# underactuated/HSLabs

Measured on AMD Instinct MI355X. Metric: batched control-loop steps/sec (hexapod.xml, 18-DoF) at 1/2/4/8 MI355X, higher is better.
Workload: dtype f64

## Files before the change

hslabs_amd/api.py:

```python
from __future__ import annotations

import ctypes
from dataclasses import dataclass, field

import numpy as np

from . import capi

GAIT_DTYPE = np.dtype([
    ("torso_pos", "<f8", (3,)), ("torso_angles", "<f8", (3,)), ("step_duration", "<f8"),
    ("period", "<f8"), ("step_length", "<f8"), ("step_height", "<f8"), ("curvature", "<f8"),
    ("foot_shift", "<f8"), ("foot_shift_type", "<i4"), ("rec_transform_flag", "<i4"),
    ("rec_transl", "<f8", (3,)), ("rec_eas", "<f8", (3,)), ("reserved", "<f8", (5,)),
])
assert GAIT_DTYPE.itemsize == 192


def _require(ok: bool, msg: str) -> None:
    if not ok:
        raise ValueError(msg)

SWEEP_NAMES = ("step_duration", "period", "step_length", "step_height")


# ... 141 lines not shown
    def __del__(self):
        try:
            if self.handle:
                capi.load().hs_model_free(self.handle)
                self.handle = None
        except Exception:
            pass


def limb_tile_launches() -> int:
    return int(capi.load().hs_limb_tile_launches())


def limb_tile_plan_launches() -> int:
    return int(capi.load().hs_limb_tile_plan_launches())


def limb_launches() -> int:
    return int(capi.load().hs_limb_launches())


def limb_deferred() -> int:
    d = ctypes.c_int64()
    capi.check(capi.load().hs_limb_stats(None, ctypes.byref(d)), "hs_limb_stats")
    return int(d.value)


def params_array(params) -> np.ndarray:
    if isinstance(params, np.ndarray) and params.dtype == GAIT_DTYPE:
        return np.ascontiguousarray(params)
# ... 724 lines not shown
```

hslabs_amd/capi.py:

```python
from __future__ import annotations

import ctypes
import hashlib
import os

from . import build as _build

ABI_VERSION = 16

HS_OK = 0
HS_FLAG_RANK_RETRY = 1
HS_FLAG_FULL_RANK = 2
HS_FLAG_LOOP_EXHAUST = 4
HS_FLAG_NAN = 8
HS_FLAG_UNREACH = 16
HS_FLAG_NO_CONTACT = 32
HS_FLAG_GENERAL = 64
HS_FLAG_NEAR_RANK = 256
HS_FLAG_DEPENDENT = 512
HS_PREC_F64 = 0
HS_PREC_F32 = 1
HS_SOLVE_AUTO = 0
HS_SOLVE_REFERENCE = 1
KEY_MIN_STEP_LENGTH = 1e-3
# ... 1 lines not shown

EXPORTS = [
    "hs_model_load", "hs_model_load_ex", "hs_model_free", "hs_model_get_dims", "hs_pgs_config_read",
    "hs_run", "hs_run_steps", "hs_run_calls", "hs_run_pd", "hs_run_forces", "hs_run_forces_calls", "hs_mixed_create", "hs_mixed_free",
    "hs_mixed_get_dims", "hs_complete_traj", "hs_traj_save", "hs_run_forces_host",
    "hs_run_mixed", "hs_run_mixed_steps", "hs_run_mixed_calls", "hs_run_host", "hs_best_key_cot", "hs_best_key_encode",
    "hs_best_key_decode", "hs_last_error", "hs_abi_version",
    "hs_sim_default_params", "hs_sim_reset", "hs_sim_step", "hs_sim_create", "hs_sim_advance", "hs_sim_get_state",
    "hs_sim_free", "hs_sim_trial", "hs_sim_trial_summary", "hs_sim_set_trial", "hs_sim_get_trial_state",
    "hs_sim_config", "hs_sim_track_push", "hs_sim_probe", "hs_sim_estimate_workspace",
    "hs_batch_create", "hs_batch_set_params", "hs_batch_run", "hs_batch_run_device", "hs_select_best",
    "hs_batch_best_key_device", "hs_batch_free", "hs_comm_unique_id", "hs_comm_init", "hs_comm_free", "hs_comm_size",
    "hs_comm_reduce_best", "hs_select_best_comm", "hs_pergen_rec", "hs_pergen_rec_host", "hs_model_lik",
    "hs_model_lik_host", "hs_model_fk", "hs_model_fk_host", "hs_model_get_node", "hs_model_set_torso_penalty",
    "hs_model_get_torso_penalty", "hs_model_limb_lane", "hs_limb_launches", "hs_limb_tile_launches", "hs_limb_stats",
    "hs_limb_tile_plan_launches",
]
EXPORTS_B = ["hs_sim_regress_B", "hs_sim_estimate_B"]
HS_FLAG_LIK_FAILED = 128
SIM_BODY_STRIDE = 13
HS_TRIAL_RUNNING = -1
HS_TRIAL_SURVIVED = -2


class GaitParamsC(ctypes.Structure):

    _fields_ = [
        ("torso_pos", ctypes.c_double * 3),
        ("torso_angles", ctypes.c_double * 3),
        ("step_duration", ctypes.c_double),
        ("period", ctypes.c_double),
# ... 208 lines not shown
    L.hs_pergen_rec_host.argtypes = [vp, ctypes.POINTER(GaitParamsC), ctypes.c_int32, dp, ctypes.c_int32, dp]
    L.hs_model_lik.argtypes = [vp, ctypes.c_int32, vp, ctypes.c_int32, vp, vp, vp]
    L.hs_model_lik_host.argtypes = [vp, ctypes.c_int32, dp, ctypes.c_int32, dp, u32p]
    L.hs_model_fk.argtypes = [vp, ctypes.c_int32, vp, ctypes.c_int32, vp, vp, vp]
    L.hs_model_fk_host.argtypes = [vp, ctypes.c_int32, dp, ctypes.c_int32, dp, dp]
    L.hs_model_get_node.argtypes = [vp, ctypes.c_int32, ctypes.POINTER(NodeInfoC)]
    L.hs_last_error.argtypes = []
    L.hs_last_error.restype = ctypes.c_char_p
    L.hs_model_limb_lane.argtypes = [vp, ctypes.POINTER(ctypes.c_int32)]
    L.hs_limb_launches.argtypes = []
    L.hs_limb_launches.restype = ctypes.c_int64
    L.hs_limb_tile_launches.argtypes = []
    L.hs_limb_tile_launches.restype = ctypes.c_int64
    L.hs_limb_tile_plan_launches.argtypes = []
    L.hs_limb_tile_plan_launches.restype = ctypes.c_int64
    L.hs_limb_stats.argtypes = [ctypes.POINTER(ctypes.c_int64), ctypes.POINTER(ctypes.c_int64)]
    L.hs_abi_version.argtypes = []
    L.hs_abi_version.restype = ctypes.c_int
    if L.hs_abi_version() != ABI_VERSION:
        raise HSError("libhslabs ABI version mismatch")
    _lib = L
    return L


def check(rc: int, what: str = "") -> None:
    if rc != HS_OK:
        msg = load().hs_last_error().decode(errors="replace")
        raise HSError(f"{what}: {msg} (rc={rc})")
```

hslabs_amd/csrc/hs_capi.cpp:

```cpp
#include <hip/hip_runtime.h>

#include <algorithm>
#include <atomic>
#include <cmath>
#include <cstdio>
#include <cstdlib>
#include <cstring>
#include <fstream>
#include <mutex>
#include <string>
#include <vector>

#include "hs_internal.h"

namespace {

thread_local std::string g_err;

int fail(int code, const std::string& msg) {
  g_err = msg;
  return code;
}

}
// ... 252 lines not shown
    if (e != hipSuccess) return hip_fail(e, "hipEventRecord");
  }
  if (key_reduce) {
    hs_run_args r = c;
    r.best_key = a.best_key;
    r.accumulate = 1;
    const int le = k.launch_fused_reduce(r, cx.total_mass, cx.rollout_mass, nullptr, 0);
    if (le != 0) return hip_fail((hipError_t)le, "kernel launch (best key)");
  }
  return HS_OK;
}

std::atomic<int64_t> g_limb_launches{0};
std::atomic<int64_t> g_limb_tile_launches{0};
std::atomic<int64_t> g_limb_tile_plan_launches{0};
#define HS_ONLINE_MAX_H 64

bool env_switch(const char* name, bool on_by_default) {
  const char* e = getenv(name);
  if (!e) return on_by_default;
  return on_by_default ? e[0] != '0' : e[0] == '1';
}

enum class step_route {
  ROLLOUT,
  ONLINE_DEFER,
  LIMB_ONLINE,
  FUSED,
  LIMB_FUSED,
};
// ... 19 lines not shown
#endif
bool limb_tile(step_route rt, const hs_run_args& a, int32_t n) {
  if (rt != step_route::LIMB_FUSED || !env_switch("HS_LIMB_TILE", true)) return false;
  if (const char* e = getenv("HS_LIMB_TILE_MIN")) {
    char* end = nullptr;
    const long min_n = strtol(e, &end, 10);
    if (end != e && *end == '\0' && min_n >= 1) return n >= min_n;
  }
  const int32_t idle = HS_TILE_SLOTS * limb_tile_count(n) - n;
  return a.precision != HS_PREC_F32 && n >= HS_LIMB_TILE_MIN_STEPS && 32 * idle <= n;
}
int32_t limb_tile_plan_mode() {
  if (!env_switch("HS_LIMB_TILE_PLAN", true)) return 0;
  const char* e = getenv("HS_LIMB_TILE_PLAN");
  return e && e[0] == '2' ? 2 : 1;
}

#ifndef HS_FUSED_WAVES
#define HS_FUSED_WAVES 524288
#endif
#ifndef HS_FUSED_MAX_STEPS
#define HS_FUSED_MAX_STEPS 256
#endif
#ifndef HS_FUSED_RESERVE_STEPS
#define HS_FUSED_RESERVE_STEPS 1024
#endif
int32_t fused_chunk(const hs::launch_map& mp) {
  return std::max(1, std::min(HS_FUSED_MAX_STEPS, HS_FUSED_WAVES / std::max(1, mp.n_waves)));
}

// ... 48 lines not shown
  int le = launch_setup(cx, c, mp);
  mp.red_total_mass = cx.total_mass;
  mp.red_rollout_mass = cx.rollout_mass;
  mp.red_key_steps = r.key_steps;
  hipStream_t st = (hipStream_t)a.stream;
  for (int32_t i = 0; le == 0 && i < n_chunks; i++) {
    const int64_t s0 = online ? 0 : (int64_t)i * CHUNK;
    const bool last = i + 1 == n_chunks;
    if (online) c.k0 = (int32_t)(((int64_t)a.k0 + (int64_t)i * a.horizon) % a.n_t);
    mp.fused_s0 = (int32_t)s0;
    mp.fused_n = (int32_t)std::min<int64_t>(CHUNK, S - s0);
    mp.fix_mode = hs::FIX_DEFER;
    mp.fix_count = fix_counts + i;
    mp.fix_reduce = 0;
    mp.limb_tile = limb_tile(rt, a, mp.fused_n);
    hipError_t e = kernel_events ? hipEventRecord((hipEvent_t)kernel_events[2 * i], st) : hipSuccess;
    if (e != hipSuccess) return hip_fail(e, "hipEventRecord");
    int32_t planned = 0;
    le = limb ? k.launch_limb(cx.d_topo, c, cx.ws, mp, limb_tile_plan_mode(), &planned)
              : k.launch_fused(cx.d_topo, c, cx.ws, mp);
    g_limb_launches += limb;
    g_limb_tile_launches += mp.limb_tile;
    g_limb_tile_plan_launches += planned;
    if (le != 0) break;
    mp.fix_mode = hs::FIX_SOLVE;
    mp.fix_reduce = a.work_cot && a.solve_mode == HS_SOLVE_AUTO && (online || last);
    mp.fix_barrier = barrier_ok ? fix_counts + n_chunks + i : nullptr;
    mp.red_n_steps = (int32_t)S;
    mp.red_best_key = last ? r.best_key : nullptr;
    le = k.launch_fused(cx.d_topo, c, cx.ws, mp);
    if (le == 0 && kernel_events) e = hipEventRecord((hipEvent_t)kernel_events[2 * i + 1], st);
    if (e != hipSuccess) return hip_fail(e, "hipEventRecord");
  }
  if (le == 0 && !mp.fix_reduce) le = k.launch_fused_reduce(r, cx.total_mass, cx.rollout_mass, work, (int32_t)S);
  if (le != 0) return hip_fail((hipError_t)le, "kernel launch");
  return HS_OK;
}

// ... 16 lines not shown
}

extern "C" {

int hs_abi_version(void) { return HSLABS_ABI_VERSION; }

int hs_model_limb_lane(hs_model_t m, int32_t* ok) {
  if (!m || !ok) return fail(HS_E_ARG, "null argument");
  *ok = m->host.limb_lane_ok;
  return HS_OK;
}

int64_t hs_limb_launches(void) { return g_limb_launches.load(); }
int64_t hs_limb_tile_launches(void) { return g_limb_tile_launches.load(); }
int64_t hs_limb_tile_plan_launches(void) { return g_limb_tile_plan_launches.load(); }

int hs_limb_stats(int64_t* launches, int64_t* deferred) {
  if (launches) *launches = g_limb_launches.load();
  if (deferred) {
    unsigned long long n[2] = {0, 0};
    hipError_t e = (hipError_t)hs::kernels_f64.limb_deferred(&n[0]);
    if (e == hipSuccess) e = (hipError_t)hs::kernels_f32.limb_deferred(&n[1]);
    if (e != hipSuccess) return hip_fail(e, "hs_limb_stats");
    *deferred = (int64_t)(n[0] + n[1]);
  }
  return HS_OK;
}

const char* hs_last_error(void) { return g_err.c_str(); }

// ... 186 lines not shown
          (hipError_t)cx.pools->fused_fix.get(a->stream, (fix_bytes(n_chunks, CHUNK, mp) + gwb - 1) / gwb, &fix);
      if (e != hipSuccess) return hip_fail(e, "hipMalloc(forces fixup items)");
    }
    fix_counts = (int32_t*)fix;
    fix_carve(fix, n_chunks, mp);
    mp.prep_unit = 8;
  }
  int le = launch_setup(cx, c, mp);
  for (int64_t s0 = 0, ci = 0; le == 0 && s0 < S; s0 += CHUNK, ci++) {
    mp.fused_s0 = (int32_t)s0;
    mp.fused_n = (int32_t)std::min<int64_t>(CHUNK, S - s0);
    if (limb) {
      mp.fix_count = fix_counts + ci;
      mp.fix_mode = hs::FIX_DEFER;
      mp.limb_tile = limb_tile(step_route::LIMB_FUSED, *a, mp.fused_n);
      int32_t planned = 0;
      le = k.launch_limb(cx.d_topo, c, cx.ws, mp, limb_tile_plan_mode(), &planned);
      g_limb_launches++;
      g_limb_tile_launches += mp.limb_tile;
      g_limb_tile_plan_launches += planned;
      if (le != 0) break;
      mp.fix_mode = hs::FIX_SOLVE;
      mp.fix_reduce = 0;
      le = k.launch_fused(cx.d_topo, c, cx.ws, mp);
      mp.fix_mode = hs::FIX_NONE;
    } else {
      le = k.launch_fused(cx.d_topo, c, cx.ws, mp);
    }
  }
  if (le != 0) return hip_fail((hipError_t)le, "kernel launch");
// ... 1241 lines not shown
```

hslabs_amd/csrc/hs_internal.h:

```cpp
#pragma once
#include <cstddef>
#include <mutex>
#include <string>
#include <vector>

#include "../../include/hslabs.h"
#include "hs_simtopo.h"
#include "hs_limb_tile.h"
#include "hs_topo.h"

struct hs_sim_probe_kargs {
  hs_sim_args sim;
  int32_t m, pad;
  const double* tau0;
  const double* dtau;
  double* config_out;
  double* tau_out;
  double* body_out;
  uint32_t* seed_out;
};

namespace hs {

int set_error(int code, const std::string& msg);
// ... 25 lines not shown
  int32_t setup_only;
  int32_t fix_mode;
  int32_t* fix_count;
  int32_t* fix_items;
  int32_t fix_n_counts;
  int32_t fix_reduce, red_key_steps, red_n_steps;
  int32_t* fix_barrier;
  double red_total_mass;
  const double* red_rollout_mass;
  uint64_t* red_best_key;
  int32_t ktab_n, ktab_lo, ktab_nl, ttab_n;
  int32_t prep_unit;
  const int32_t *limb_model, *limb_rollouts, *limb_slots;
  int32_t limb_waves;
  int32_t limb_tile;
};

size_t solve_workspace_bytes();
void ktab_range(int32_t k0, int32_t n_t, int32_t horizon, int64_t n_calls, int32_t* lo, int32_t* n_table,
                int32_t* n_ttab);
launch_map single_model_map(const hs_topo& t, int32_t n_rollouts);

struct kernels {
  size_t (*general_workspace_bytes)();
  int (*launch_rollouts)(const hs_topo* d_topo, const hs_run_args& a, void* workspace, const launch_map& mp);
  int (*launch_fused)(const hs_topo* d_topo, const hs_run_args& a, void* workspace, const launch_map& mp);
  int (*launch_limb)(const hs_topo* d_topo, const hs_run_args& a, void* workspace, const launch_map& mp,
                     int32_t tile_plan, int32_t* tile_planned);
  int (*launch_fused_reduce)(const hs_run_args& a, double total_mass, const double* rollout_mass,
                             const void* work_steps, int32_t n_steps);
// ... 67 lines not shown
```

hslabs_amd/csrc/hs_kernels.hip:

```cpp
#include <hip/hip_runtime.h>

#include <cfloat>
#include <cstdint>
#include <type_traits>

#ifndef HS_REAL_IS_FLOAT
#define HS_REAL_IS_FLOAT 0
#endif
#include "hs_internal.h"
#include "hs_math.h"

namespace {

using namespace hsd;

#ifndef HS_CURVED_LDS
#define HS_CURVED_LDS HS_REAL_IS_FLOAT
#endif
#ifndef HS_PRELOAD
#define HS_PRELOAD (!HS_REAL_IS_FLOAT)
#endif
#ifndef HS_KTE_PRELOAD
#define HS_KTE_PRELOAD (!HS_REAL_IS_FLOAT)
#endif
// ... 172 lines not shown
template <class T>
__device__ inline bool near_thr(T v, T t, T band) { return v >= t / band && v <= t * band; }

__device__ inline real* outp(double* p) { return reinterpret_cast<real*>(p); }
__device__ inline const real* inp(const double* p) { return reinterpret_cast<const real*>(p); }

template <class G>
__device__ inline void gsync() {
  if constexpr (G::SHARED) wave_sync();
  else __syncthreads();
}

#ifdef HS_STAMPS
__device__ unsigned long long g_stamps[4096][32];
__device__ unsigned int g_stamp_base;
#define STAMP(slot)                                                                                    \
  do {                                                                                                 \
    const unsigned r_ = blockIdx.x - g_stamp_base;                                                     \
    if (threadIdx.x == 0 && r_ < 4096u) g_stamps[r_][slot] = __builtin_amdgcn_s_memtime();             \
  } while (0)
#define RSTAMP(slot)                                                                                   \
  do {                                                                                                 \
    const unsigned r_ = blockIdx.x - g_stamp_base;                                                     \
    if (threadIdx.x == 0 && r_ < 4096u) g_stamps[r_][slot] = __builtin_amdgcn_s_memrealtime();         \
  } while (0)
#else
#define STAMP(slot) do {} while (0)
#define RSTAMP(slot) do {} while (0)
#endif

#ifdef HS_DBG
__device__ double g_dbg[1 << 22];
__device__ inline int* dbg_rows() {
  __shared__ int r[8];
// ... 2861 lines not shown
extern "C" int hs_debug_read_dbg(double* out, int n) {
  if (n > (1 << 22)) n = 1 << 22;
  return (int)hipMemcpyFromSymbol(out, HIP_SYMBOL(g_dbg), sizeof(double) * n, 0, hipMemcpyDeviceToHost);
}
#endif

#if defined(HS_STAMPS) && !HS_REAL_IS_FLOAT
extern "C" int hs_debug_read_stamps(unsigned long long* out, int n_rows) {
  if (n_rows > 4096) n_rows = 4096;
  return (int)hipMemcpyFromSymbol(out, HIP_SYMBOL(g_stamps), sizeof(unsigned long long) * 32 * n_rows, 0,
                                  hipMemcpyDeviceToHost);
}
extern "C" int hs_debug_set_stamp_base(unsigned int base) {
  return (int)hipMemcpyToSymbol(HIP_SYMBOL(g_stamp_base), &base, sizeof(base), 0, hipMemcpyHostToDevice);
}
extern "C" int hs_debug_clear_stamps() {
  static unsigned long long zero[4096][32];
  return (int)hipMemcpyToSymbol(HIP_SYMBOL(g_stamps), zero, sizeof(zero), 0, hipMemcpyHostToDevice);
}
#endif

namespace hs {

static size_t general_workspace_bytes() { return sizeof(RolloutWS); }

static int limb_deferred(unsigned long long* out) {
  return (int)hipMemcpyFromSymbol(out, HIP_SYMBOL(g_limb_deferred), sizeof(unsigned long long), 0,
                                  hipMemcpyDeviceToHost);
}

// ... 82 lines not shown
  if (mp.max_parts <= 18) launch_nm<18>(d_topo, a, ws, m, st);
  else if (mp.max_parts <= 22) launch_nm<22>(d_topo, a, ws, m, st);
  else launch_nm<HS_NMAX>(d_topo, a, ws, m, st);
  return (int)hipGetLastError();
}

static int launch_limb(const hs_topo* d_topo, const hs_run_args& a, void* workspace, const launch_map& mp,
                       int32_t tile_plan, int32_t* tile_planned) {
  if (tile_planned) *tile_planned = 0;
  if (a.n_rollouts <= 0 || mp.fused_n <= 0) return 0;
  hipStream_t st = (hipStream_t)a.stream;
  RolloutWS* ws = (RolloutWS*)workspace;
  launch_map m = mp;
  m.fused_w = mp.limb_rollouts ? mp.limb_waves : (a.n_rollouts + LGR - 1) / LGR;
  const int vsteps = mp.limb_tile ? HS_TILE_SLOTS * limb_tile_count(mp.fused_n) : mp.fused_n;
  const dim3 grid((unsigned)((int64_t)m.fused_w * vsteps));
  const int nm = mp.max_parts <= 18 ? 18 : (mp.max_parts <= 22 ? 22 : HS_NMAX);
  limb_tile_plan_arg plan = {};
  if (mp.limb_tile && tile_plan && mp.fused_n <= HS_TILE_PLAN_STEPS && mp.fused_h >= 1 && a.n_t >= 1 && a.k0 >= 0 &&
      mp.fused_s0 >= 0) {
    const limb_tile_launch L = {mp.fused_n, mp.fused_s0, mp.fused_h, a.k0, a.n_t, mp.ktab_nl > 0 ? mp.ktab_nl : HS_LMAX};
    bool planned = true;
    if (tile_plan == 2) {
      int row[HS_TILE_PLAN_STEPS];
      limb_tile_rows(L, row);
      limb_tile_chain_fill(row, L.n, plan.step);
    } else {
      planned = limb_tile_plan(L, plan.step);
    }
    if (planned) plan.n_slots = vsteps;
    if (tile_planned) *tile_planned = planned;
// ... 47 lines not shown
```

hslabs_amd/csrc/hs_limb.h:

```cpp

#ifndef HS_LIMB_GROUP
#define HS_LIMB_GROUP HS_FUSED_GROUP
#endif
#ifndef HS_LIMB_WAVES
#define HS_LIMB_WAVES 2
#endif
#ifndef HS_LIMB_WAVES_F32
#define HS_LIMB_WAVES_F32 HS_LIMB_WAVES
#endif

constexpr int LG = 8;
constexpr int LGR = WAVE / LG;

__device__ unsigned long long g_limb_deferred;

template <int NM, bool FORCES = false>
struct LimbLds {
  real g[NM][6];
  real a[6];
  real wd[HS_NMAX];
  real p[FORCES ? NM : 1][3];
};

__device__ inline real grp_get(real v, int src) { return __shfl(v, src); }
// ... 169 lines not shown
      }
    }
    for (int e = 0; e < 6; e++) tD[m][e] = Dp[e];
    for (int i = 0; i < 3; i++) tg[m][i] = g[i];
  }
#pragma unroll
  for (int e = 0; e < 6; e++) Dp6[e] = (tD[0][e] + tD[1][e]) + (tD[2][e] + real(0));
#pragma unroll
  for (int i = 0; i < 3; i++) gc[i] = (tg[0][i] + tg[1][i]) + (tg[2][i] + real(0));
}

template <int NM>
__device__ __attribute__((always_inline)) inline void limb_forces(const hs_topo* T, const hs_run_args& a,
                                                                  const hs::launch_map& mp, LimbLds<NM, true>& S, bool limb,
                                                                  int l, int L, int gbase, int nl, bool live, int b,
                                                                  int fstep, int s_glob, const real* o,
                                                                  const real (&Jp)[3][3], const real (&Jz)[3][3],
                                                                  const real (&Pc)[3][3], const real* fp,
                                                                  const real (&xt)[3][3], bool bad, bool big) {
  const int n = T->n;
#ifdef HS_DBG
  const int dbg_r = live ? b * a.horizon + s_glob : -1;
#define FDBG(slot, val, n_)                                                                                      \
  do {                                                                                                           \
    if (HS_DBG == (n_) && dbg_r >= 0 && (size_t)dbg_r * 32 + (slot) < (1u << 22)) g_dbg[(size_t)dbg_r * 32 + (slot)] = (double)(val); \
  } while (0)
#else
#define FDBG(slot, val, n_) do {} while (0)
#endif
  real ts[9];
#pragma unroll
// ... 31 lines not shown
      for (int e = 0; e < 27; e++) {
        const TriWalk<> t(e < 21 ? e : 0);
        real pa = e < 21 ? F.prod(t.r, t.c) : F.prod(e - 21, 9);
        real pb = e < 21 ? G.vprod(t.r, t.c) : G.vprod(e - 21, 6);
        opaque_vals<1>(&pa);
        opaque_vals<1>(&pb);
        vl[e] = (e < 21) ? pb - pa : pb + pa;
      }
    }
  }
  const bool fast = !grp_any(limb && !okB, gbase);
  if (!fast || grp_any(big, gbase)) {
    if (l == 0 && live) {
      atomicAdd(&g_limb_deferred, 1ull);
      const int it = atomicAdd(mp.fix_count, 1);
      mp.fix_items[2 * it] = fstep;
      mp.fix_items[2 * it + 1] = b;
    }
    return;
  }
  real kv[27];
#pragma unroll
  for (int e = 0; e < 27; e++) {
    const real v = limb ? vl[e] : real(0);
    real s = real(0) + v;
    for (int k = 1; k < nl; k++) {
      const real prev = dpp_r<0x111>(s);
      if (l >= 1) s = prev + v;
    }
    const real tot = grp_get(s, gbase + nl - 1);
    const real dtv = (e < 21) ? real(0) : (e < 24 ? S.a[e - 21] : S.a[e - 21]);
// ... 53 lines not shown
    return (real)__hiloint2double(hi, lo);
  } else {
    return (real)__int_as_float(__builtin_amdgcn_ds_permute(dst << 2, __float_as_int((float)v)));
  }
}

#ifdef HS_DBG
#define TDBG(slot, val, n)                                                                                       \
  do {                                                                                                           \
    if (HS_DBG == (n) && dbg_r >= 0 && (size_t)dbg_r * 32 + (slot) < (1u << 22)) g_dbg[(size_t)dbg_r * 32 + (slot)] = (double)(val); \
  } while (0)
#else
#define TDBG(slot, val, n) do {} while (0)
#endif

template <bool FORCES>
__device__ __attribute__((always_inline)) inline void limb_tile_kd(
    const hs_topo* T_, real (&outer)[36][LGR * HS_LMAX], hs_link (&links)[HS_LMAX][3], const RolloutWS& W, bool straight,
    const real* u, real v, int lane, int nl, bool limb, int L, bool live, int row0, const real* tv, const real* o,
    real inv, real dt, real (&g3)[3][6], real (&Jp)[3][3], real (&Jz)[3][3], real* fp, bool& contact, bool& own,
    real* gown, real* jvel, real (&Pc)[3][3], real* Pown, bool& bad, bool& big, int dbg_r) {
  (void)dbg_r;
  const int grp = lane >> 3, l = lane & 7;
  const int rprev = __shfl(row0, (lane + WAVE - LG) & (WAVE - 1)), rnext = __shfl(row0, (lane + LG) & (WAVE - 1));
  const uint64_t lv = __ballot(live);
  const bool lprev = grp > 0 && ((lv >> ((lane - LG) & (WAVE - 1))) & 1);
  const bool lnext = grp < LGR - 1 && ((lv >> ((lane + LG) & (WAVE - 1))) & 1);
  const bool shm = live && lprev && rprev + 2 == row0;
  const bool shp = live && lnext && rnext == row0 + 2;
  uint32_t M = 0;
  {
    const uint64_t bm = __ballot(live && !shm), bp = __ballot(live && !shp);
#pragma unroll
    for (int g = 0; g < LGR; g++)
      M |= (uint32_t)((bm >> (LG * g)) & 1) << (2 * g) | (uint32_t)((bp >> (LG * g)) & 1) << (2 * g + 1);
  }
  const int nreq = __popc(M);
// ... 160 lines not shown
    for (int r = 0; r < 5; r += 2)
#pragma unroll
      for (int kk = 0; kk < 3; kk++) big |= sincos_big(W.ktab[row0 + r][L][kk]);
#pragma unroll
    for (int kk = 0; kk < 3; kk++) {
      if constexpr (FORCES) break;
      real dd = W.ktab[row0 + 3][L][kk] - W.ktab[row0 + 1][L][kk];
      if (dd > kPi) dd -= 2 * kPi;
      else if (dd < -kPi) dd += 2 * kPi;
      jvel[kk] = dd / (2 * dt);
    }
  }
}
#undef TDBG

template <int NM, bool FORCES, bool TILE = false, class... PLAN>
__global__ __launch_bounds__(WAVE, HS_REAL_IS_FLOAT ? HS_LIMB_WAVES_F32 : HS_LIMB_WAVES) void hs_limb_kernel(const hs_topo* __restrict__ T0, hs_run_args a,
                                                                      RolloutWS* __restrict__ rws, hs::launch_map mp, PLAN... plan) {
  static_assert(sizeof...(PLAN) == (TILE ? 1 : 0), "the tile mapping takes the launch's plan, the packed mapping nothing");
  __shared__ union {
    struct {
      real outer[36][LGR * HS_LMAX];
      hs_link links[HS_LMAX][3];
    } k;
    LimbLds<NM, FORCES> g[LGR];
  } sh;
  LimbLds<NM, FORCES>* lds = sh.g;
  int fstep = 0, q = (int)blockIdx.x;
  fused_coords<HS_LIMB_GROUP>((int)blockIdx.x, mp.fused_w, TILE ? HS_TILE_SLOTS * limb_tile_count(mp.fused_n) : mp.fused_n,
                              fstep, q);
  const hs_topo* __restrict__ T = mp.limb_model ? T0 + mp.limb_model[q] : T0;
  {
    const uint64_t* src = reinterpret_cast<const uint64_t*>(&T->link[0][0]);
    uint64_t* dst = reinterpret_cast<uint64_t*>(&sh.k.links[0][0]);
    constexpr int NW = sizeof(sh.k.links) / sizeof(uint64_t);
    for (int e = (int)threadIdx.x; e < NW; e += WAVE) dst[e] = src[e];
    wave_sync();
  }
  RSTAMP(16);
  STAMP(15);
  const int lane = (int)threadIdx.x, grp = lane >> 3, l = lane & 7, gbase = lane & ~7;
  const int rslot = q * LGR + (TILE ? fstep % LGR : grp);
  const int b = mp.limb_rollouts ? mp.limb_rollouts[rslot] : rslot;
  bool live = b >= 0 && b < a.n_rollouts;
  if constexpr (TILE) {
    if (!live) return;
    const int slot0 = HS_TILE_SLOTS * (fstep / LGR), ls = limb_tile_plan_step(plan..., slot0 + grp, mp.fused_n);
    live = ls >= 0;
    fstep = live ? ls : limb_tile_plan_step(plan..., slot0, mp.fused_n);
  }
  const int bb = live || TILE ? b : (mp.limb_rollouts ? mp.limb_rollouts[q * LGR] : a.n_rollouts - 1);
  LimbLds<NM, FORCES>& S = lds[grp];
  const int ol = grp * HS_LMAX + (l < HS_LMAX ? l : 0);
  const int s_glob = mp.fused_s0 + fstep, call = s_glob / mp.fused_h;
  const int k0 = (int)(((int64_t)a.k0 + (int64_t)call * mp.fused_h) % a.n_t) + s_glob % mp.fused_h;
  const int row0 = k0 - mp.ktab_lo;
  const int nl = T->n_limbs, nmj = T->nmj;
  const bool limb = l < nl, tlane = l == LG - 1;
  const int L = limb ? l : 0;
  const RolloutWS& W = rws[bb];
  const hs_gait_params& gp = a.params[bb];
  const bool straight = (real)gp.curvature == 0 && !gp.rec_transform_flag;
  const real dt = W.st.dt;
  const real v = W.st.v;
  const NodeK n0 = load_nodek(T, 0);
  const real u[3] = {n0.Jp(0, 0), n0.Jp(1, 0), n0.Jp(2, 0)};
  real tv[5];
#pragma unroll
  for (int k = 0; k < 5; k += 2) tv[k] = W.t_tab[row0 + k] * v;
  real o[3];
  if (straight) {
    for (int i = 0; i < 3; i++) o[i] = fma(tv[2], u[i], W.kf.torso[i]);
  } else {
    mulp(load34r(W.ktor[row0 + 2] + 6), n0.com, o);
  }
  const real inv = real(1) / (2 * dt);
#ifdef HS_DBG
  const int dbg_r = live ? b * a.horizon + s_glob : -1;
#define LDBG(slot, val, n)                                                                                       \
  do {                                                                                                           \
    if (HS_DBG == (n) && dbg_r >= 0 && (size_t)dbg_r * 32 + (slot) < (1u << 22)) g_dbg[(size_t)dbg_r * 32 + (slot)] = (double)(val); \
  } while (0)
#else
#define LDBG(slot, val, n) do {} while (0)
#endif

  real g0[6];
  {
    BodyS tb[3];
#pragma unroll
    for (int k = 0; k < 3; k++) {
      if (straight) tb[k] = body_straight(W.kf.torso, u, tv[2 * k]);
      else tb[k] = body_frame(load34r(W.ktor[row0 + 2 * k] + 6), n0.com);
    }
    part_dyn((real)T->mass[0], inv, tb[0].P, tb[1].P, tb[2].P, tb[0].U, tb[1].U, tb[2].U, g0);
    part_g(tb[1].P, o, g0);
  }
  STAMP(0);
  real g3[3][6];
  real Jp[3][3], Jz[3][3], fp[3];
  bool contact = false;
  bool own = false;
  real gown[6];
  real jvel[3];
  real Pc[3][3], Pown[3];
  bool bad = false, big = false;
  const hs_topo* const T_ = T;
  if constexpr (TILE) {
    limb_tile_kd<FORCES>(T_, sh.k.outer, sh.k.links, W, straight, u, v, lane, nl, limb, L, live, row0, tv, o, inv, dt, g3,
                         Jp, Jz, fp, contact, own, gown, jvel, Pc, Pown, bad, big, live ? b * a.horizon + s_glob : -1);
  } else if (limb) {
    const int row = row0;
    own = T->limb_own_n[L] > 0;
    BodyS om, op, oc;
    {
      real P[3][3], U[3][3];
      const hs_topo* Ts = opaque_s(T);
      limb_outer(Ts, sh.k.links[L], limb_frame(Ts, L, straight, own, W, row, u, tv[0], om), W.ktab[row][L], P, U, big);
#pragma unroll
      for (int kk = 0; kk < 3; kk++)
#pragma unroll
        for (int j = 0; j < 3; j++) {
          sh.k.outer[3 * kk + j][ol] = P[kk][j];
          sh.k.outer[9 + 3 * kk + j][ol] = U[kk][j];
        }
// ... 143 lines not shown
    const int nk = T->node[0].nkids;
    for (int kk = 0; kk < HS_CMAX; kk++) {
      if (kk >= nk) break;
      const int c = T->node[0].kids[kk];
      for (int j = 0; j < 3; j++) { F[j] += S.g[c][j]; V[j] += S.g[c][3 + j]; }
    }
    const real d[3] = {0, 0, 0};
    V[0] -= d[1] * F[2] - d[2] * F[1];
    V[1] -= d[2] * F[0] - d[0] * F[2];
    V[2] -= d[0] * F[1] - d[1] * F[0];
    for (int j = 0; j < 3; j++) { S.a[j] = F[j]; S.a[3 + j] = V[j]; }
  }
  wave_sync();

  STAMP(5);
  if constexpr (FORCES) {
    limb_forces<NM>(T, a, mp, S, limb, l, L, gbase, nl, live, b, fstep, s_glob, o, Jp, Jz, Pc, fp, xt, bad, big);
    return;
  }
  const int fiL = T->link[L][2].foot;
  const uint32_t cm = grp_or((limb && contact) ? 1u << fiL : 0u);
  const int nc = __popc(cm);
  const bool mine = limb && contact;
  if (limb) LDBG(24 + fiL, fp[2], 25);
  int src = 0;
  for (int L2 = 0; L2 < nl; L2++) {
    const int f2 = T->link[L2][2].foot;
    if (((cm >> f2) & 1) && __popc(cm & ((1u << f2) - 1)) == l) src = L2;
  }
  src += gbase;
  const bool slot = l < nc;
  bool defer = grp_any(big, gbase);
// ... 215 lines not shown
      }
    }
    defer |= !ok;
    nearf |= lnear;
    if (mine && ok) {
      const int rk = __popc(cm & ((1u << fiL) - 1));
      for (int i = 0; i < 3; i++) y3[i] = rk == 0 ? y[i] : y[3 + i];
      opaque_vals<3>(y3);
    }
  }
  STAMP(8);
  if (defer) {
    if (l == 0 && live) {
      atomicAdd(&g_limb_deferred, 1ull);
      const int it = atomicAdd(mp.fix_count, 1);
      mp.fix_items[2 * it] = fstep;
      mp.fix_items[2 * it + 1] = mp.limb_slots ? mp.limb_slots[rslot] : b;
    }
    return;
  }

  const size_t orow = (size_t)b * a.horizon + s_glob;
  bool nan = false;
  if (limb) {
#pragma unroll
    for (int kk = 0; kk < 3; kk++) {
      const int hh = T->link[L][kk].hinge;
      real d[3], yy[3];
#pragma unroll
      for (int rr = 0; rr < 3; rr++) {
        d[rr] = Jp[kk][rr] - fp[rr];
// ... 34 lines not shown
  if (l == 0 && live) {
    uint32_t flags = 0;
    if (nc == 0) flags |= HS_FLAG_NO_CONTACT;
    if (nc == 1) flags |= HS_FLAG_FULL_RANK;
    if (nearf) flags |= HS_FLAG_NEAR_RANK;
    if (any_nan) flags |= HS_FLAG_NAN;
    if (any_bad) flags |= HS_FLAG_UNREACH;
    if (a.flags) a.flags[orow] = flags;
    real work_dt = real(0);
    for (int jj = 0; jj < nmj; jj++) work_dt += S.wd[jj];
    reinterpret_cast<real*>(mp.fused_work)[(size_t)s_glob * a.n_rollouts + b] = work_dt;
  }
  STAMP(9);
  RSTAMP(17);
}
```

hslabs_amd/csrc/hs_limb_tile.h:

```cpp
#pragma once

#include <stdint.h>

#if defined(__HIP__)
#define HS_TILE_FN __host__ __device__ inline
#else
#define HS_TILE_FN inline
#endif

constexpr int HS_TILE_SLOTS = 8;

HS_TILE_FN int limb_tile_count(int n) { return (n + HS_TILE_SLOTS - 1) / HS_TILE_SLOTS; }

HS_TILE_FN int limb_tile_step(int slot, int n) {
  const int n_even = (n + 1) / 2;
  if (slot < 0 || slot >= n) return -1;
  return slot < n_even ? 2 * slot : 2 * (slot - n_even) + 1;
}

constexpr int HS_TILE_PLAN_STEPS = 256;

struct limb_tile_plan_arg {
  int32_t n_slots;
  int16_t step[HS_TILE_PLAN_STEPS];
};
HS_TILE_FN int limb_tile_plan_step(const limb_tile_plan_arg& p, int slot, int n) {
  if (p.n_slots == 0) return limb_tile_step(slot, n);
  return slot >= 0 && slot < p.n_slots ? p.step[slot] : -1;
}

struct limb_tile_launch {
  int n, s0, h, k0, n_t, n_limbs;
// ... 117 lines not shown
```

include/hslabs.h:

```cpp
#ifndef HSLABS_H
#define HSLABS_H
#include <stddef.h>
#include <stdint.h>
#ifdef __cplusplus
extern "C" {
#endif

#define HSLABS_ABI_VERSION 16

enum {
  HS_OK = 0,
  HS_E_ARG = -1,
  HS_E_IO = -2,
  HS_E_PARSE = -3,
  HS_E_TOPOLOGY = -4,
  HS_E_NOLIK = -5,
  HS_E_DEVICE = -6,
  HS_E_NOTFOUND = -7
};

#define HS_FLAG_RANK_RETRY   1u
#define HS_FLAG_FULL_RANK    2u
#define HS_FLAG_LOOP_EXHAUST 4u
#define HS_FLAG_NAN          8u
// ... 296 lines not shown
typedef struct hs_sim_s* hs_sim_t;
int hs_sim_create(hs_model_t model, const hs_gait_params* params, int32_t n_rollouts, const hs_sim_params* sim_params,
                  double t0, hs_sim_t* out);
int hs_sim_advance(hs_sim_t sim, int32_t n_steps, double* tau_cmd, double* q_meas, double* torso, int32_t* n_contacts,
                   double* normal_force);
int hs_sim_get_state(hs_sim_t sim, double* body, int32_t* tsi);
int hs_sim_set_trial(hs_sim_t sim, int32_t open_loop, double torque_limit, int32_t kick_every, int32_t kick_phase,
                     const double* kick_dv_host, double hc, int32_t check_from, int32_t check_until);
int hs_sim_get_trial_state(hs_sim_t sim, int32_t* state_host);
void hs_sim_free(hs_sim_t sim);

int hs_model_limb_lane(hs_model_t model, int32_t* ok);
int64_t hs_limb_launches(void);
int64_t hs_limb_tile_launches(void);
int64_t hs_limb_tile_plan_launches(void);
int hs_limb_stats(int64_t* launches, int64_t* deferred);

const char* hs_last_error(void);
int hs_abi_version(void);

#ifdef __cplusplus
}
#endif
#endif
```

Measured before the change: 934.8 million.

## Loop several limb tiles per wavefront in the tiled limb kernel

The tiled limb kernel can now process a chunk of consecutive tiles inside one wavefront instead of launching one wavefront per tile, for f64 non-force launches. A host rule picks the chunk length so that enough waves stay resident. Per-rollout setup (link table copy into LDS, rollout lookup, gait flags, node-0 axis) is hoisted out of the per-tile body, and kernel args are re-read via opaque pointers to limit register pressure. The trade-off is fewer waves and less parallelism, plus a link table kept outside the LDS union, which raises LDS use per wave.

```diff
diff --git a/hslabs_amd/api.py b/hslabs_amd/api.py
--- a/hslabs_amd/api.py
+++ b/hslabs_amd/api.py
@@ -179,6 +179,10 @@
 
 def limb_tile_plan_launches() -> int:
     return int(capi.load().hs_limb_tile_plan_launches())
+
+
+def limb_tile_loop_launches() -> int:
+    return int(capi.load().hs_limb_tile_loop_launches())
 
 
 def limb_launches() -> int:
diff --git a/hslabs_amd/capi.py b/hslabs_amd/capi.py
--- a/hslabs_amd/capi.py
+++ b/hslabs_amd/capi.py
@@ -39,7 +39,7 @@
     "hs_comm_reduce_best", "hs_select_best_comm", "hs_pergen_rec", "hs_pergen_rec_host", "hs_model_lik",
     "hs_model_lik_host", "hs_model_fk", "hs_model_fk_host", "hs_model_get_node", "hs_model_set_torso_penalty",
     "hs_model_get_torso_penalty", "hs_model_limb_lane", "hs_limb_launches", "hs_limb_tile_launches", "hs_limb_stats",
-    "hs_limb_tile_plan_launches",
+    "hs_limb_tile_plan_launches", "hs_limb_tile_loop_launches",
 ]
 EXPORTS_B = ["hs_sim_regress_B", "hs_sim_estimate_B"]
 HS_FLAG_LIK_FAILED = 128
@@ -278,6 +278,8 @@
     L.hs_limb_tile_launches.restype = ctypes.c_int64
     L.hs_limb_tile_plan_launches.argtypes = []
     L.hs_limb_tile_plan_launches.restype = ctypes.c_int64
+    L.hs_limb_tile_loop_launches.argtypes = []
+    L.hs_limb_tile_loop_launches.restype = ctypes.c_int64
     L.hs_limb_stats.argtypes = [ctypes.POINTER(ctypes.c_int64), ctypes.POINTER(ctypes.c_int64)]
     L.hs_abi_version.argtypes = []
     L.hs_abi_version.restype = ctypes.c_int
diff --git a/hslabs_amd/csrc/hs_capi.cpp b/hslabs_amd/csrc/hs_capi.cpp
--- a/hslabs_amd/csrc/hs_capi.cpp
+++ b/hslabs_amd/csrc/hs_capi.cpp
@@ -290,6 +290,7 @@
 std::atomic<int64_t> g_limb_launches{0};
 std::atomic<int64_t> g_limb_tile_launches{0};
 std::atomic<int64_t> g_limb_tile_plan_launches{0};
+std::atomic<int64_t> g_limb_tile_loop_launches{0};
 #define HS_ONLINE_MAX_H 64
 
 bool env_switch(const char* name, bool on_by_default) {
@@ -339,6 +340,23 @@
   if (!env_switch("HS_LIMB_TILE_PLAN", true)) return 0;
   const char* e = getenv("HS_LIMB_TILE_PLAN");
   return e && e[0] == '2' ? 2 : 1;
+}
+#ifndef HS_LIMB_TILE_LOOP_TILES
+#define HS_LIMB_TILE_LOOP_TILES 5
+#endif
+#ifndef HS_LIMB_TILE_LOOP_ROUNDS
+#define HS_LIMB_TILE_LOOP_ROUNDS 4
+#endif
+constexpr int64_t HS_RESIDENT_LIMB_WAVES = 2048;
+int32_t limb_tile_loop(const hs_run_args& a, int32_t n) {
+  const int32_t nt = limb_tile_count(n);
+  if (a.precision == HS_PREC_F32) return 1;
+  if (const char* e = getenv("HS_LIMB_TILE_LOOP")) {
+    char* end = nullptr;
+    const long tl = strtol(e, &end, 10);
+    if (end != e && *end == '\0' && tl >= 1) return (int32_t)std::min<long>(tl, HS_TILE_PLAN_STEPS);
+  }
+  return limb_tile_loop_rule(nt, a.n_rollouts, HS_LIMB_TILE_LOOP_TILES, HS_LIMB_TILE_LOOP_ROUNDS * HS_RESIDENT_LIMB_WAVES);
 }
 
 #ifndef HS_FUSED_WAVES
@@ -417,6 +435,7 @@
     mp.fix_count = fix_counts + i;
     mp.fix_reduce = 0;
     mp.limb_tile = limb_tile(rt, a, mp.fused_n);
+    mp.limb_tile_loop = mp.limb_tile ? limb_tile_loop(a, mp.fused_n) : 1;
     hipError_t e = kernel_events ? hipEventRecord((hipEvent_t)kernel_events[2 * i], st) : hipSuccess;
     if (e != hipSuccess) return hip_fail(e, "hipEventRecord");
     int32_t planned = 0;
@@ -425,6 +444,7 @@
     g_limb_launches += limb;
     g_limb_tile_launches += mp.limb_tile;
     g_limb_tile_plan_launches += planned;
+    g_limb_tile_loop_launches += mp.limb_tile && std::min(mp.limb_tile_loop, limb_tile_count(mp.fused_n)) > 1;
     if (le != 0) break;
     mp.fix_mode = hs::FIX_SOLVE;
     mp.fix_reduce = a.work_cot && a.solve_mode == HS_SOLVE_AUTO && (online || last);
@@ -471,6 +491,7 @@
 int64_t hs_limb_launches(void) { return g_limb_launches.load(); }
 int64_t hs_limb_tile_launches(void) { return g_limb_tile_launches.load(); }
 int64_t hs_limb_tile_plan_launches(void) { return g_limb_tile_plan_launches.load(); }
+int64_t hs_limb_tile_loop_launches(void) { return g_limb_tile_loop_launches.load(); }
 
 int hs_limb_stats(int64_t* launches, int64_t* deferred) {
   if (launches) *launches = g_limb_launches.load();
@@ -687,6 +708,7 @@
       mp.fix_count = fix_counts + ci;
       mp.fix_mode = hs::FIX_DEFER;
       mp.limb_tile = limb_tile(step_route::LIMB_FUSED, *a, mp.fused_n);
+      mp.limb_tile_loop = 1;
       int32_t planned = 0;
       le = k.launch_limb(cx.d_topo, c, cx.ws, mp, limb_tile_plan_mode(), &planned);
       g_limb_launches++;
diff --git a/hslabs_amd/csrc/hs_internal.h b/hslabs_amd/csrc/hs_internal.h
--- a/hslabs_amd/csrc/hs_internal.h
+++ b/hslabs_amd/csrc/hs_internal.h
@@ -63,6 +63,7 @@
   const int32_t *limb_model, *limb_rollouts, *limb_slots;
   int32_t limb_waves;
   int32_t limb_tile;
+  int32_t limb_tile_loop;
 };
 
 size_t solve_workspace_bytes();
diff --git a/hslabs_amd/csrc/hs_kernels.hip b/hslabs_amd/csrc/hs_kernels.hip
--- a/hslabs_amd/csrc/hs_kernels.hip
+++ b/hslabs_amd/csrc/hs_kernels.hip
@@ -210,10 +210,12 @@
 #ifdef HS_STAMPS
 __device__ unsigned long long g_stamps[4096][32];
 __device__ unsigned int g_stamp_base;
+__device__ int g_stamp_iter;
+#define HS_STAMP_GATE true
 #define STAMP(slot)                                                                                    \
   do {                                                                                                 \
     const unsigned r_ = blockIdx.x - g_stamp_base;                                                     \
-    if (threadIdx.x == 0 && r_ < 4096u) g_stamps[r_][slot] = __builtin_amdgcn_s_memtime();             \
+    if (threadIdx.x == 0 && r_ < 4096u && (HS_STAMP_GATE)) g_stamps[r_][slot] = __builtin_amdgcn_s_memtime(); \
   } while (0)
 #define RSTAMP(slot)                                                                                   \
   do {                                                                                                 \
@@ -3105,6 +3107,9 @@
 extern "C" int hs_debug_set_stamp_base(unsigned int base) {
   return (int)hipMemcpyToSymbol(HIP_SYMBOL(g_stamp_base), &base, sizeof(base), 0, hipMemcpyHostToDevice);
 }
+extern "C" int hs_debug_set_stamp_iter(int iter) {
+  return (int)hipMemcpyToSymbol(HIP_SYMBOL(g_stamp_iter), &iter, sizeof(iter), 0, hipMemcpyHostToDevice);
+}
 extern "C" int hs_debug_clear_stamps() {
   static unsigned long long zero[4096][32];
   return (int)hipMemcpyToSymbol(HIP_SYMBOL(g_stamps), zero, sizeof(zero), 0, hipMemcpyHostToDevice);
@@ -3217,7 +3222,9 @@
   launch_map m = mp;
   m.fused_w = mp.limb_rollouts ? mp.limb_waves : (a.n_rollouts + LGR - 1) / LGR;
   const int vsteps = mp.limb_tile ? HS_TILE_SLOTS * limb_tile_count(mp.fused_n) : mp.fused_n;
-  const dim3 grid((unsigned)((int64_t)m.fused_w * vsteps));
+  m.limb_tile_loop = mp.limb_tile_loop < 1 || mp.tau_in || HS_REAL_IS_FLOAT ? 1 : mp.limb_tile_loop;
+  const int wsteps = mp.limb_tile ? HS_TILE_SLOTS * limb_tile_chunks(limb_tile_count(mp.fused_n), m.limb_tile_loop) : mp.fused_n;
+  const dim3 grid((unsigned)((int64_t)m.fused_w * wsteps));
   const int nm = mp.max_parts <= 18 ? 18 : (mp.max_parts <= 22 ? 22 : HS_NMAX);
   limb_tile_plan_arg plan = {};
   if (mp.limb_tile && tile_plan && mp.fused_n <= HS_TILE_PLAN_STEPS && mp.fused_h >= 1 && a.n_t >= 1 && a.k0 >= 0 &&
diff --git a/hslabs_amd/csrc/hs_limb.h b/hslabs_amd/csrc/hs_limb.h
--- a/hslabs_amd/csrc/hs_limb.h
+++ b/hslabs_amd/csrc/hs_limb.h
@@ -207,7 +207,7 @@
 __device__ __attribute__((always_inline)) inline void limb_forces(const hs_topo* T, const hs_run_args& a,
                                                                   const hs::launch_map& mp, LimbLds<NM, true>& S, bool limb,
                                                                   int l, int L, int gbase, int nl, bool live, int b,
-                                                                  int fstep, int s_glob, const real* o,
+                                                                  int s_glob, const real* o,
                                                                   const real (&Jp)[3][3], const real (&Jz)[3][3],
                                                                   const real (&Pc)[3][3], const real* fp,
                                                                   const real (&xt)[3][3], bool bad, bool big) {
@@ -269,7 +269,7 @@
     if (l == 0 && live) {
       atomicAdd(&g_limb_deferred, 1ull);
       const int it = atomicAdd(mp.fix_count, 1);
-      mp.fix_items[2 * it] = fstep;
+      mp.fix_items[2 * it] = s_glob - mp.fused_s0;
       mp.fix_items[2 * it + 1] = b;
     }
     return;
@@ -353,13 +353,18 @@
 #define TDBG(slot, val, n) do {} while (0)
 #endif
 
+#ifdef HS_STAMPS
+#undef HS_STAMP_GATE
+#define HS_STAMP_GATE stamp_on
+#endif
 template <bool FORCES>
 __device__ __attribute__((always_inline)) inline void limb_tile_kd(
     const hs_topo* T_, real (&outer)[36][LGR * HS_LMAX], hs_link (&links)[HS_LMAX][3], const RolloutWS& W, bool straight,
     const real* u, real v, int lane, int nl, bool limb, int L, bool live, int row0, const real* tv, const real* o,
     real inv, real dt, real (&g3)[3][6], real (&Jp)[3][3], real (&Jz)[3][3], real* fp, bool& contact, bool& own,
-    real* gown, real* jvel, real (&Pc)[3][3], real* Pown, bool& bad, bool& big, int dbg_r) {
+    real* gown, real* jvel, real (&Pc)[3][3], real* Pown, bool& bad, bool& big, int dbg_r, bool stamp_on) {
   (void)dbg_r;
+  (void)stamp_on;
   const int grp = lane >> 3, l = lane & 7;
   const int rprev = __shfl(row0, (lane + WAVE - LG) & (WAVE - 1)), rnext = __shfl(row0, (lane + LG) & (WAVE - 1));
   const uint64_t lv = __ballot(live);
@@ -550,69 +555,102 @@
 }
 #undef TDBG
 
-template <int NM, bool FORCES, bool TILE = false, class... PLAN>
-__global__ __launch_bounds__(WAVE, HS_REAL_IS_FLOAT ? HS_LIMB_WAVES_F32 : HS_LIMB_WAVES) void hs_limb_kernel(const hs_topo* __restrict__ T0, hs_run_args a,
-                                                                      RolloutWS* __restrict__ rws, hs::launch_map mp, PLAN... plan) {
-  static_assert(sizeof...(PLAN) == (TILE ? 1 : 0), "the tile mapping takes the launch's plan, the packed mapping nothing");
-  __shared__ union {
+
+template <int NM, bool FORCES, bool LOOP>
+struct LimbShared {
+  union {
     struct {
       real outer[36][LGR * HS_LMAX];
       hs_link links[HS_LMAX][3];
     } k;
     LimbLds<NM, FORCES> g[LGR];
-  } sh;
-  LimbLds<NM, FORCES>* lds = sh.g;
-  int fstep = 0, q = (int)blockIdx.x;
-  fused_coords<HS_LIMB_GROUP>((int)blockIdx.x, mp.fused_w, TILE ? HS_TILE_SLOTS * limb_tile_count(mp.fused_n) : mp.fused_n,
-                              fstep, q);
-  const hs_topo* __restrict__ T = mp.limb_model ? T0 + mp.limb_model[q] : T0;
-  {
-    const uint64_t* src = reinterpret_cast<const uint64_t*>(&T->link[0][0]);
-    uint64_t* dst = reinterpret_cast<uint64_t*>(&sh.k.links[0][0]);
-    constexpr int NW = sizeof(sh.k.links) / sizeof(uint64_t);
-    for (int e = (int)threadIdx.x; e < NW; e += WAVE) dst[e] = src[e];
-    wave_sync();
-  }
-  RSTAMP(16);
-  STAMP(15);
-  const int lane = (int)threadIdx.x, grp = lane >> 3, l = lane & 7, gbase = lane & ~7;
-  const int rslot = q * LGR + (TILE ? fstep % LGR : grp);
-  const int b = mp.limb_rollouts ? mp.limb_rollouts[rslot] : rslot;
-  bool live = b >= 0 && b < a.n_rollouts;
+  };
+  __device__ hs_link (&links())[HS_LMAX][3] { return k.links; }
+};
+template <int NM, bool FORCES>
+struct LimbShared<NM, FORCES, true> {
+  union {
+    struct {
+      real outer[36][LGR * HS_LMAX];
+    } k;
+    LimbLds<NM, FORCES> g[LGR];
+  };
+  hs_link tl[HS_LMAX][3];
+  __device__ hs_link (&links())[HS_LMAX][3] { return tl; }
+};
+static_assert(sizeof(LimbShared<HS_NMAX, false, true>) <= 20480, "a looping wavefront's LDS: 8 per CU's 160 KB");
+
+struct LimbHead {
+  int lane;
+  int rslot, b;
+  bool live;
+  bool straight;
+  const RolloutWS* W;
+  real u[3];
+};
+
+template <class P>
+__device__ inline const P* opaque_u(const P* p) {
+  using cptr = const __attribute__((address_space(4))) P*;
+  cptr q = (cptr)p;
+  asm volatile("" : "+s"(q));
+  return (const P*)q;
+}
+
+template <class P>
+__device__ inline const P& opaque_k(const P& r) {
+  using kptr = const __attribute__((address_space(4))) P*;
+  kptr q = (kptr)&r;
+  asm volatile("" : "+s"(q));
+  return *(const P*)q;
+}
+
+template <int NM, bool FORCES, bool TILE, bool LOOP, class... PLAN>
+__device__ __attribute__((always_inline)) inline void limb_step(LimbShared<NM, FORCES, LOOP>& sh, const hs_topo* __restrict__ T,
+                                                                const hs_run_args& a0, const hs::launch_map& mp0,
+                                                                const LimbHead& h, int fstep, bool stamp_on,
+                                                                const PLAN&... plan) {
+  (void)stamp_on;
+  STAMP(23);
+  int lane = h.lane;
+  if constexpr (LOOP) {
+    asm volatile("" : "+v"(lane));
+    T = opaque_u(T);
+  }
+  const int grp = lane >> 3, l = lane & 7, gbase = lane & ~7, rslot = h.rslot, b = h.b;
+  const int nl = T->n_limbs, nmj = T->nmj;
+  const bool limb = l < nl, tlane = l == LG - 1, straight = h.straight;
+  const int L = limb ? l : 0;
+  const real u[3] = {h.u[0], h.u[1], h.u[2]};
+  bool live = h.live;
   if constexpr (TILE) {
-    if (!live) return;
-    const int slot0 = HS_TILE_SLOTS * (fstep / LGR), ls = limb_tile_plan_step(plan..., slot0 + grp, mp.fused_n);
+    const int slot0 = HS_TILE_SLOTS * fstep, ls = limb_tile_plan_step(plan..., slot0 + grp, mp0.fused_n);
     live = ls >= 0;
-    fstep = live ? ls : limb_tile_plan_step(plan..., slot0, mp.fused_n);
-  }
-  const int bb = live || TILE ? b : (mp.limb_rollouts ? mp.limb_rollouts[q * LGR] : a.n_rollouts - 1);
-  LimbLds<NM, FORCES>& S = lds[grp];
-  const int ol = grp * HS_LMAX + (l < HS_LMAX ? l : 0);
-  const int s_glob = mp.fused_s0 + fstep, call = s_glob / mp.fused_h;
-  const int k0 = (int)(((int64_t)a.k0 + (int64_t)call * mp.fused_h) % a.n_t) + s_glob % mp.fused_h;
-  const int row0 = k0 - mp.ktab_lo;
-  const int nl = T->n_limbs, nmj = T->nmj;
-  const bool limb = l < nl, tlane = l == LG - 1;
-  const int L = limb ? l : 0;
-  const RolloutWS& W = rws[bb];
-  const hs_gait_params& gp = a.params[bb];
-  const bool straight = (real)gp.curvature == 0 && !gp.rec_transform_flag;
+    fstep = live ? ls : limb_tile_plan_step(plan..., slot0, mp0.fused_n);
+  }
+  const RolloutWS* Wp = h.W;
+  if constexpr (LOOP) Wp = opaque_u(Wp);
+  const RolloutWS& W = *Wp;
   const real dt = W.st.dt;
   const real v = W.st.v;
-  const NodeK n0 = load_nodek(T, 0);
-  const real u[3] = {n0.Jp(0, 0), n0.Jp(1, 0), n0.Jp(2, 0)};
+  const real inv = real(1) / (2 * dt);
+  LimbLds<NM, FORCES>& S = sh.g[grp];
+  const int ol = grp * HS_LMAX + (l < HS_LMAX ? l : 0);
+  const int s_glob = mp0.fused_s0 + fstep, call = s_glob / mp0.fused_h;
+  const int k0 = (int)(((int64_t)a0.k0 + (int64_t)call * mp0.fused_h) % a0.n_t) + s_glob % mp0.fused_h;
+  const int row0 = k0 - mp0.ktab_lo;
   real tv[5];
 #pragma unroll
   for (int k = 0; k < 5; k += 2) tv[k] = W.t_tab[row0 + k] * v;
   real o[3];
+  const real com0[3] = {(real)T->node[0].com[0], (real)T->node[0].com[1], (real)T->node[0].com[2]};
   if (straight) {
     for (int i = 0; i < 3; i++) o[i] = fma(tv[2], u[i], W.kf.torso[i]);
   } else {
-    mulp(load34r(W.ktor[row0 + 2] + 6), n0.com, o);
-  }
-  const real inv = real(1) / (2 * dt);
+    mulp(load34r(W.ktor[row0 + 2] + 6), com0, o);
+  }
 #ifdef HS_DBG
-  const int dbg_r = live ? b * a.horizon + s_glob : -1;
+  const int dbg_r = live ? b * a0.horizon + s_glob : -1;
 #define LDBG(slot, val, n)                                                                                       \
   do {                                                                                                           \
     if (HS_DBG == (n) && dbg_r >= 0 && (size_t)dbg_r * 32 + (slot) < (1u << 22)) g_dbg[(size_t)dbg_r * 32 + (slot)] = (double)(val); \
@@ -627,7 +665,7 @@
 #pragma unroll
     for (int k = 0; k < 3; k++) {
       if (straight) tb[k] = body_straight(W.kf.torso, u, tv[2 * k]);
-      else tb[k] = body_frame(load34r(W.ktor[row0 + 2 * k] + 6), n0.com);
+      else tb[k] = body_frame(load34r(W.ktor[row0 + 2 * k] + 6), com0);
     }
     part_dyn((real)T->mass[0], inv, tb[0].P, tb[1].P, tb[2].P, tb[0].U, tb[1].U, tb[2].U, g0);
     part_g(tb[1].P, o, g0);
@@ -643,8 +681,9 @@
   bool bad = false, big = false;
   const hs_topo* const T_ = T;
   if constexpr (TILE) {
-    limb_tile_kd<FORCES>(T_, sh.k.outer, sh.k.links, W, straight, u, v, lane, nl, limb, L, live, row0, tv, o, inv, dt, g3,
-                         Jp, Jz, fp, contact, own, gown, jvel, Pc, Pown, bad, big, live ? b * a.horizon + s_glob : -1);
+    limb_tile_kd<FORCES>(T_, sh.k.outer, sh.links(), W, straight, u, v, lane, nl, limb, L, live, row0, tv, o, inv, dt, g3,
+                         Jp, Jz, fp, contact, own, gown, jvel, Pc, Pown, bad, big, live ? b * a0.horizon + s_glob : -1,
+                         stamp_on);
   } else if (limb) {
     const int row = row0;
     own = T->limb_own_n[L] > 0;
@@ -818,8 +857,10 @@
   wave_sync();
 
   STAMP(5);
+  const hs_run_args& a = LOOP ? opaque_k(a0) : a0;
+  const hs::launch_map& mp = LOOP ? opaque_k(mp0) : mp0;
   if constexpr (FORCES) {
-    limb_forces<NM>(T, a, mp, S, limb, l, L, gbase, nl, live, b, fstep, s_glob, o, Jp, Jz, Pc, fp, xt, bad, big);
+    limb_forces<NM>(T, a, mp, S, limb, l, L, gbase, nl, live, b, s_glob, o, Jp, Jz, Pc, fp, xt, bad, big);
     return;
   }
   const int fiL = T->link[L][2].foot;
@@ -1065,7 +1106,7 @@
     if (l == 0 && live) {
       atomicAdd(&g_limb_deferred, 1ull);
       const int it = atomicAdd(mp.fix_count, 1);
-      mp.fix_items[2 * it] = fstep;
+      mp.fix_items[2 * it] = s_glob - mp.fused_s0;
       mp.fix_items[2 * it + 1] = mp.limb_slots ? mp.limb_slots[rslot] : b;
     }
     return;
@@ -1130,3 +1171,76 @@
   STAMP(9);
   RSTAMP(17);
 }
+#undef LDBG
+#ifdef HS_STAMPS
+#undef HS_STAMP_GATE
+#define HS_STAMP_GATE true
+#endif
+
+struct LimbTileArgs {
+  const hs_topo* T0;
+  hs_run_args a;
+  RolloutWS* rws;
+  hs::launch_map mp;
+  limb_tile_plan_arg plan;
+};
+
+template <int NM, bool FORCES, bool TILE = false, class... PLAN>
+__global__ __launch_bounds__(WAVE, HS_REAL_IS_FLOAT ? HS_LIMB_WAVES_F32 : HS_LIMB_WAVES) void hs_limb_kernel(const hs_topo* __restrict__ T0, hs_run_args a,
+                                                                      RolloutWS* __restrict__ rws, hs::launch_map mp, PLAN... plan) {
+  static_assert(sizeof...(PLAN) == (TILE ? 1 : 0), "the tile mapping takes the launch's plan, the packed mapping nothing");
+  static_assert(!TILE || (std::is_same<PLAN, limb_tile_plan_arg>::value && ...), "LimbTileArgs holds a limb_tile_plan_arg");
+  static_assert(offsetof(LimbTileArgs, a) == 8 && offsetof(LimbTileArgs, rws) == 8 + sizeof(hs_run_args) &&
+                    offsetof(LimbTileArgs, mp) == 16 + sizeof(hs_run_args) &&
+                    offsetof(LimbTileArgs, plan) == 16 + sizeof(hs_run_args) + sizeof(hs::launch_map) &&
+                    alignof(hs_run_args) == 8 && alignof(hs::launch_map) == 8,
+                "LimbTileArgs: the kernel argument segment packs the arguments in order at their alignment");
+  constexpr bool LOOP = TILE && !FORCES && !HS_REAL_IS_FLOAT;
+  __shared__ LimbShared<NM, FORCES, LOOP> sh;
+  int fstep = 0, q = (int)blockIdx.x;
+  const int nt = TILE ? limb_tile_count(mp.fused_n) : 0, tl = LOOP ? mp.limb_tile_loop : 1;
+  fused_coords<HS_LIMB_GROUP>((int)blockIdx.x, mp.fused_w, TILE ? HS_TILE_SLOTS * limb_tile_chunks(nt, tl) : mp.fused_n, fstep,
+                              q);
+  const hs_topo* __restrict__ T = mp.limb_model ? T0 + mp.limb_model[q] : T0;
+  {
+    const uint64_t* src = reinterpret_cast<const uint64_t*>(&T->link[0][0]);
+    uint64_t* dst = reinterpret_cast<uint64_t*>(&sh.links()[0][0]);
+    constexpr int NW = sizeof(hs_link[HS_LMAX][3]) / sizeof(uint64_t);
+    for (int e = (int)threadIdx.x; e < NW; e += WAVE) dst[e] = src[e];
+    wave_sync();
+  }
+  RSTAMP(16);
+  STAMP(15);
+  LimbHead h;
+  h.lane = (int)threadIdx.x;
+  h.rslot = q * LGR + (TILE ? fstep % LGR : h.lane >> 3);
+  h.b = mp.limb_rollouts ? mp.limb_rollouts[h.rslot] : h.rslot;
+  h.live = h.b >= 0 && h.b < a.n_rollouts;
+  if (TILE && !h.live) return;
+  const int bb = h.live ? h.b : (mp.limb_rollouts ? mp.limb_rollouts[q * LGR] : a.n_rollouts - 1);
+  h.W = &rws[bb];
+  const hs_gait_params& gp = a.params[bb];
+  h.straight = (real)gp.curvature == 0 && !gp.rec_transform_flag;
+  {
+    const NodeK n0 = load_nodek(T, 0);
+    for (int i = 0; i < 3; i++) h.u[i] = n0.Jp(i, 0);
+  }
+  if constexpr (LOOP) {
+    const int c = fstep / LGR;
+    for (int t0 = limb_tile_chunk_first(c, tl), t = t0, te = limb_tile_chunk_end(c, tl, nt); t < te; t++) {
+      using kptr = const __attribute__((address_space(4))) LimbTileArgs*;
+      kptr ka = (kptr)__builtin_amdgcn_kernarg_segment_ptr();
+      asm volatile("" : "+s"(ka));
+      const LimbTileArgs& k = *(const LimbTileArgs*)ka;
+#ifdef HS_STAMPS
+      const bool stamp_on = t - t0 == g_stamp_iter;
+#else
+      const bool stamp_on = true;
+#endif
+      limb_step<NM, FORCES, true, true>(sh, T, k.a, k.mp, h, t, stamp_on, k.plan);
+      wave_sync();
+    }
+  } else {
+    limb_step<NM, FORCES, TILE, false>(sh, T, a, mp, h, TILE ? fstep / LGR : fstep, true, plan...);
+  }
+}
diff --git a/hslabs_amd/csrc/hs_limb_tile.h b/hslabs_amd/csrc/hs_limb_tile.h
--- a/hslabs_amd/csrc/hs_limb_tile.h
+++ b/hslabs_amd/csrc/hs_limb_tile.h
@@ -16,6 +16,24 @@
   const int n_even = (n + 1) / 2;
   if (slot < 0 || slot >= n) return -1;
   return slot < n_even ? 2 * slot : 2 * (slot - n_even) + 1;
+}
+
+HS_TILE_FN int limb_tile_chunks(int nt, int tl) {
+  tl = tl < 1 ? 1 : tl;
+  return (nt + tl - 1) / tl;
+}
+HS_TILE_FN int limb_tile_chunk_first(int c, int tl) { return c * (tl < 1 ? 1 : tl); }
+HS_TILE_FN int limb_tile_chunk_end(int c, int tl, int nt) {
+  const int e = limb_tile_chunk_first(c, tl) + (tl < 1 ? 1 : tl);
+  return e < nt ? e : nt;
+}
+
+HS_TILE_FN int limb_tile_loop_rule(int nt, int64_t n_rollouts, int tiles, int64_t min_waves) {
+  int tl = tiles < nt ? tiles : nt;
+  while (tl > 1 && (int64_t)limb_tile_chunks(nt, tl) * n_rollouts < min_waves) tl--;
+  if (tl < 1) return 1;
+  const int nc = limb_tile_chunks(nt, tl);
+  return (nt + nc - 1) / nc;
 }
 
 constexpr int HS_TILE_PLAN_STEPS = 256;
diff --git a/include/hslabs.h b/include/hslabs.h
--- a/include/hslabs.h
+++ b/include/hslabs.h
@@ -334,6 +334,7 @@
 int64_t hs_limb_launches(void);
 int64_t hs_limb_tile_launches(void);
 int64_t hs_limb_tile_plan_launches(void);
+int64_t hs_limb_tile_loop_launches(void);
 int hs_limb_stats(int64_t* launches, int64_t* deferred);
 
 const char* hs_last_error(void);
```

After: 984.6 million, median of 6. 5.3% higher.
